# pudnax/voidin

Measured on AMD Instinct MI355X. Metric: M instances culled+compacted/sec, higher is better.
Workload: dtype f32; 1 GPU; configs[2]: 10M synthetic AABB instances, cull + prefix-sum compaction (BASELINE.md §3 distribution, model.rs camera); instances_per_gpu=10000000, instances_total=10000000, n_meshes=16, distribution=baseline, parallelism=single GPU

## Files before the change

### voidin_amd/csrc/cull.hip

```cpp
#include "vd_common.hpp"

#include <math.h>

namespace {

constexpr int kWave = 64;
constexpr int kBlock = 256;
constexpr int kWavesPerBlock = kBlock / kWave;
constexpr int kInstBytes = 144;
constexpr int kSlabBytes = kWave * kInstBytes;
constexpr int kChunksPerLane = kSlabBytes / (kWave * 16);



typedef unsigned int u32x4 __attribute__((ext_vector_type(4)));

struct CullCamera {
    float view[16];
    float frustum[4];
    float znear, zfar;
};

struct MeshRec { float mnx, mny, mnz; unsigned index_count; float mxx, mxy, mxz; unsigned base_index; int vertex_offset; };

// ... 276 lines not shown
    const float v0 = (0.5f - ny_hi * 0.5f) * H - 0.5f, v1 = (0.5f - ny_lo * 0.5f) * H + 0.5f;
    if (!(u1 >= 0.0f && v1 >= 0.0f && u0 < W && v0 < H)) return false;
    const unsigned x0 = (unsigned)floorf(fmaxf(u0, 0.0f)), x1 = (unsigned)floorf(fminf(u1, W - 1.0f));
    const unsigned y0 = (unsigned)floorf(fmaxf(v0, 0.0f)), y1 = (unsigned)floorf(fminf(v1, H - 1.0f));
    const unsigned span = max(x1 - x0, y1 - y0);
    const unsigned lvl = min(span ? 32u - (unsigned)__clz((int)span) : 0u, hz.n_levels - 1u);
    const float* t = hz.base + hz.off[lvl];
    const unsigned lw = ((hz.width - 1u) >> lvl) + 1u;
    const unsigned ax = x0 >> lvl, bx = x1 >> lvl, ay = y0 >> lvl, by = y1 >> lvl;
    const float h0 = fminf(t[(size_t)ay * lw + ax], t[(size_t)ay * lw + bx]);
    const float h1 = fminf(t[(size_t)by * lw + ax], t[(size_t)by * lw + bx]);
    const float hmin = fminf(h0, h1);
    const float depth = (cam.p32 - cam.p22 * dn) / dn;
    return depth < hmin;
}

__global__ __launch_bounds__(kBlock, 3) void occlusion_mask_kernel(OccCamera cam, HizView hz, const VdMeshInfo* __restrict__ meshes,
                                                                   unsigned n_mesh, const VdInstance* __restrict__ inst, unsigned n_inst,
                                                                   const vd_u64* __restrict__ mask_in, vd_u64* __restrict__ mask_out,
                                                                   unsigned n_wave_tiles) {
    extern __shared__ __attribute__((aligned(16))) char smem[];
    const unsigned lane = threadIdx.x & 63u, wave = threadIdx.x >> 6;
    char* slab = smem + wave * kSlabBytes;
    const unsigned waves_total = gridDim.x * kWavesPerBlock;
    u32x4 regs[kChunksPerLane];
    for (unsigned wt = blockIdx.x * kWavesPerBlock + wave; wt < n_wave_tiles; wt += waves_total) {
        const vd_u64 in = mask_in[wt];
        if (in == 0ull) {
            if (lane == 0) mask_out[wt] = 0ull;
            continue;
        }
        const size_t first = (size_t)wt * kWave;
        const unsigned n_valid = min(64u, n_inst - (unsigned)first);
        slab_fill<false>(inst, first, n_valid, lane, regs);
        slab_store(slab, lane, regs);
        vd_wave_lds_sync();
        const LaneInst li = slab_read(slab, lane);
        vd_wave_lds_sync();
        bool keep = false;
        if (lane < n_valid && ((in >> lane) & 1ull)) {
            const MeshRec m = load_mesh(meshes, min(li.mesh, n_mesh - 1u));
            keep = !is_occluded(cam, hz, m, li.T0, li.T1, li.T2, li.T3);
        }
        const unsigned long long b = __ballot(keep);
        if (lane == 0) mask_out[wt] = b;
    }
}

constexpr int kMaskRounds = 16;
template <typename IdT>
__global__ __launch_bounds__(kBlock, 3) void cull_mask_tiled_kernel(CullCamera cam, const VdMeshInfo* __restrict__ meshes,
                                                                     unsigned n_mesh, const VdInstance* __restrict__ inst,
                                                                     unsigned n_inst, vd_u64* __restrict__ mask,
                                                                     IdT* __restrict__ ids_out, unsigned n_tiles) {
    extern __shared__ __attribute__((aligned(16))) char smem[];
    const unsigned lane = threadIdx.x & 63u, wave = threadIdx.x >> 6;
    constexpr int kIdBytes = kMaskRounds * kWave * (int)sizeof(IdT);
    char* slab = smem + wave * (kSlabBytes + kIdBytes);
    IdT* s_ids = reinterpret_cast<IdT*>(slab + kSlabBytes);
    const unsigned waves_total = gridDim.x * kWavesPerBlock;
    auto valid_at = [&](size_t f) -> unsigned { return f < n_inst ? (unsigned)min((size_t)64, (size_t)n_inst - f) : 0u; };
    u32x4 regs[kChunksPerLane];
    for (unsigned t = blockIdx.x * kWavesPerBlock + wave; t < n_tiles; t += waves_total) {
        const size_t tile_first = (size_t)t * (kWave * kMaskRounds);
        slab_fill<true>(inst, tile_first, valid_at(tile_first), lane, regs);
        constexpr int kIdRows = kIdBytes / (kWave * 16);
        u32x4 old_ids[kIdRows];
        const size_t id_base0 = tile_first * sizeof(IdT);
        const bool full_tile = tile_first + (size_t)kWave * kMaskRounds <= (size_t)n_inst;
        if (full_tile) {
#pragma unroll
            for (int r = 0; r < kIdRows; ++r)
                old_ids[r] = *reinterpret_cast<const u32x4*>(reinterpret_cast<const char*>(ids_out) + id_base0 + (size_t)r * kWave * 16 + lane * 16u);
        }
        vd_u64 my_word = 0;
#pragma unroll 1
        for (int r = 0; r < kMaskRounds; ++r) {
            const size_t first = tile_first + (size_t)r * kWave;
            const unsigned n_valid = valid_at(first);
            slab_store(slab, lane, regs);
            if (r + 1 < kMaskRounds) slab_fill<true>(inst, first + kWave, valid_at(first + kWave), lane, regs);
            vd_wave_lds_sync();
            const LaneInst li = slab_read(slab, lane);
            vd_wave_lds_sync();
            const unsigned mid = min(li.mesh, n_mesh - 1u);
            const MeshRec m = load_mesh(meshes, mid);
            const bool vis = lane < n_valid && is_visible(cam, m, li.T0, li.T1, li.T2, li.T3);
            const unsigned long long b = __ballot(vis);
            if (lane == (unsigned)r) my_word = b;
            s_ids[r * kWave + lane] = (IdT)mid;
        }
        vd_wave_lds_sync();
        const size_t w0 = (size_t)t * kMaskRounds;
        const size_t n_words = ((size_t)n_inst + 63) / 64;
        if (lane < (unsigned)kMaskRounds && w0 + lane < n_words) mask[w0 + lane] = my_word;
        const size_t id_base = tile_first * sizeof(IdT);
        const size_t id_end = min((size_t)n_inst, tile_first + (size_t)kWave * kMaskRounds) * sizeof(IdT);
        char* gids = reinterpret_cast<char*>(ids_out);
        if (full_tile) {
#pragma unroll
            for (int r = 0; r < kIdRows; ++r) {
                const unsigned b0 = (unsigned)r * kWave * 16u + lane * 16u;
                const u32x4 nv = *reinterpret_cast<const u32x4*>(reinterpret_cast<const char*>(s_ids) + b0);
                const bool diff = nv.x != old_ids[r].x || nv.y != old_ids[r].y || nv.z != old_ids[r].z || nv.w != old_ids[r].w;
                if (__any(diff)) *reinterpret_cast<u32x4*>(gids + id_base + b0) = nv;
            }
        } else {
            for (unsigned b0 = lane * 16u; b0 < (unsigned)kIdBytes; b0 += kWave * 16u) {
                if (id_base + b0 + 16u <= id_end) {
                    *reinterpret_cast<u32x4*>(gids + id_base + b0) = *reinterpret_cast<const u32x4*>(reinterpret_cast<const char*>(s_ids) + b0);
                } else {
                    for (unsigned q = 0; q < 16u && id_base + b0 + q < id_end; ++q) gids[id_base + b0 + q] = reinterpret_cast<const char*>(s_ids)[b0 + q];
                }
            }
        }
        vd_wave_lds_sync();
    }
}

constexpr int kExpandGroup = 4;
constexpr int kExpandWords = 32;
constexpr int kChunkWords = kWavesPerBlock * kExpandWords;

constexpr int kScanBlock = 1024;
struct ScanState { unsigned done, epoch, pad[2]; };
__global__ __launch_bounds__(kScanBlock) void mask_scan_kernel(const vd_u64* __restrict__ mask, unsigned n_words, unsigned n_chunks,
                                                           vd_u64* chunk_entry, ScanState* state,
                                                           unsigned* __restrict__ out_count) {
    constexpr int kScanWaves = kScanBlock / kWave;
    __shared__ unsigned s_last, s_wave_sum[kScanWaves];
    const unsigned lane = threadIdx.x & 63u, wave = threadIdx.x >> 6;
    const unsigned ep = __hip_atomic_load(&state->epoch, VD_RLX_AGENT);
    const vd_u64 tag = (vd_u64)ep << 32;
    for (unsigned c = blockIdx.x * kScanWaves + wave; c < n_chunks; c += gridDim.x * kScanWaves) {
        const unsigned w = c * kChunkWords + lane;
        unsigned v = (w < n_words ? (unsigned)__popcll(mask[w]) : 0u) + (w + 64u < n_words ? (unsigned)__popcll(mask[w + 64u]) : 0u);
#pragma unroll
        for (int off = 32; off > 0; off >>= 1) v += __shfl_xor(v, off);
        if (lane == 0) __hip_atomic_store(&chunk_entry[c], tag | v, VD_RLX_AGENT);
    }
    __builtin_amdgcn_s_waitcnt(0);
    __syncthreads();
    if (threadIdx.x == 0) s_last = __hip_atomic_fetch_add(&state->done, 1u, VD_RLX_AGENT) == gridDim.x - 1u;
    __syncthreads();
    if (!s_last) return;
    const unsigned per = (n_chunks + kScanBlock - 1) / kScanBlock;
    const unsigned begin = min(threadIdx.x * per, n_chunks), end = min(begin + per, n_chunks);
    bool stuck = false;
    auto entry = [&](unsigned c) -> unsigned {
        vd_u64 e = __hip_atomic_load(&chunk_entry[c], VD_RLX_AGENT);
        unsigned spins = 0;
        while ((e >> 32) != (vd_u64)ep) {
            if (++spins > (1u << 22)) { stuck = true; return 0u; }
            __builtin_amdgcn_s_sleep(1);
            e = __hip_atomic_load(&chunk_entry[c], VD_RLX_AGENT);
        }
        return (unsigned)e;
    };
    unsigned sum = 0;
    for (unsigned c = begin; c < end; ++c) sum += entry(c);
    const bool any_stuck = __syncthreads_or(stuck ? 1 : 0) != 0;
    unsigned incl = sum;
#pragma unroll
    for (int off = 1; off < kWave; off <<= 1) {
        const unsigned t = __shfl_up(incl, off);
        if (lane >= (unsigned)off) incl += t;
    }
    if (lane == kWave - 1u) s_wave_sum[wave] = incl;
    __syncthreads();
    unsigned run = incl - sum;
    for (unsigned w = 0; w < wave; ++w) run += s_wave_sum[w];
    for (unsigned c = begin; c < end; ++c) {
        if (any_stuck) { chunk_entry[c] = tag | 0xffffffffu; continue; }
        const unsigned v = entry(c);
        chunk_entry[c] = tag | run;
        run += v;
    }
    if (threadIdx.x == kScanBlock - 1u) {
        *out_count = any_stuck ? 0xffffffffu : run;
        __hip_atomic_store(&state->done, 0u, VD_RLX_AGENT);
        __hip_atomic_store(&state->epoch, ep + 1u, VD_RLX_AGENT);
    }
}

template <typename IdT, bool TAB>
__global__ __launch_bounds__(kBlock) void expand_mask_kernel(const vd_u64* __restrict__ mask, unsigned n_words, unsigned wps,
                                                             unsigned shard_size, unsigned n_total, unsigned first_instance,
                                                             const IdT* __restrict__ mesh_ids,
                                                             const VdMeshInfo* __restrict__ meshes, unsigned n_mesh,
                                                             VdDrawIndexedIndirect* __restrict__ out,
                                                             const vd_u64* __restrict__ chunk_entry) {
    constexpr int kGroups = kExpandWords / kExpandGroup;
    constexpr unsigned kTab = TAB ? 512 : 1;
    __shared__ unsigned s_tab[kTab][3];
    constexpr int kStageBytes = kExpandGroup * 1280 + 32;
    __shared__ __attribute__((aligned(16))) char s_stage[kWavesPerBlock][kStageBytes];
    const unsigned lane = threadIdx.x & 63u, wave = threadIdx.x >> 6;
    const unsigned chunk = blockIdx.x;
    const unsigned cw0 = chunk * kChunkWords;
    const unsigned w0 = __builtin_amdgcn_readfirstlane(cw0 + wave * kExpandWords);
    unsigned base = (unsigned)chunk_entry[chunk];
    if (base == 0xffffffffu) return;
    unsigned before = 0;
    if (lane < wave * kExpandWords && cw0 + lane < n_words) before = (unsigned)__popcll(mask[cw0 + lane]);
    if (lane + 64u < wave * kExpandWords && cw0 + 64u + lane < n_words) before += (unsigned)__popcll(mask[cw0 + 64u + lane]);
    vd_u64 my_word = 0;
    if (lane < (unsigned)kExpandWords && w0 + lane < n_words) my_word = mask[w0 + lane];
    auto group_first = [&](unsigned wg, unsigned (&f)[kExpandGroup]) {
        unsigned shard = wg / wps, r = wg - shard * wps;
#pragma unroll
        for (int q = 0; q < kExpandGroup; ++q) {
            f[q] = shard * shard_size + 64u * r;
            if (++r >= wps) { r = 0u; ++shard; }
        }
    };
    unsigned ids[kExpandWords];
#pragma unroll
    for (int g = 0; g < kGroups; ++g) {
        const unsigned wg = w0 + g * kExpandGroup;
        unsigned f[kExpandGroup];
        group_first(wg, f);
#pragma unroll
        for (int q = 0; q < kExpandGroup; ++q) {
            const unsigned idx = f[q] + lane;
            ids[g * kExpandGroup + q] = (wg + q < n_words && idx < n_total) ? (unsigned)mesh_ids[idx] : 0u;
        }
    }
    if (TAB)
        for (unsigned i = threadIdx.x; i < n_mesh; i += kBlock) {
            s_tab[i][0] = meshes[i].index_count; s_tab[i][1] = meshes[i].base_index; s_tab[i][2] = (unsigned)meshes[i].vertex_offset;
        }
#pragma unroll
    for (int off = 32; off > 0; off >>= 1) before += __shfl_xor(before, off);
    base += before;
    __syncthreads();
    char* stage = s_stage[wave];
#pragma unroll
    for (int g = 0; g < kGroups; ++g) {
        const unsigned wg = w0 + g * kExpandGroup;
        vd_u64 m[kExpandGroup];
        unsigned cnt = 0;
#pragma unroll
        for (int q = 0; q < kExpandGroup; ++q) {
            const int k = g * kExpandGroup + q;
            const unsigned lo = __shfl((unsigned)my_word, k), hi = __shfl((unsigned)(my_word >> 32), k);
            m[q] = ((vd_u64)hi << 32) | lo;
            cnt += (unsigned)__popcll(m[q]);
        }
        if (cnt == 0u) continue;
        char* gbase = reinterpret_cast<char*>(out + base);
        const unsigned shift = (unsigned)(reinterpret_cast<uintptr_t>(gbase) & 15u);
        unsigned run = 0;
        unsigned first[kExpandGroup];
        group_first(wg, first);
#pragma unroll
        for (int q = 0; q < kExpandGroup; ++q) {
            unsigned mid = ids[g * kExpandGroup + q];
            if ((m[q] >> lane) & 1ull) {
                mid = min(mid, n_mesh - 1u);
                unsigned* o = reinterpret_cast<unsigned*>(stage + shift + 20u * (run + vd_mbcnt(m[q])));
                if (TAB) { o[0] = s_tab[mid][0]; o[2] = s_tab[mid][1]; o[3] = s_tab[mid][2]; }
                else { o[0] = meshes[mid].index_count; o[2] = meshes[mid].base_index; o[3] = (unsigned)meshes[mid].vertex_offset; }
                o[1] = 1u;
                o[4] = first_instance + first[q] + lane;
            }
            run += (unsigned)__popcll(m[q]);
        }
        vd_wave_lds_sync();
        const unsigned total = shift + 20u * cnt;
        char* g16 = gbase - shift;
        for (unsigned b0 = lane * 16u; b0 < total; b0 += kWave * 16u) {
            if (b0 >= shift && b0 + 16u <= total) {
                *reinterpret_cast<u32x4*>(g16 + b0) = *reinterpret_cast<const u32x4*>(stage + b0);
            } else {
                const unsigned lo_b = b0 > shift ? b0 : shift, hi_b = b0 + 16u < total ? b0 + 16u : total;
                for (unsigned b = lo_b; b < hi_b; b += 4u)
                    *reinterpret_cast<unsigned*>(g16 + b) = *reinterpret_cast<const unsigned*>(stage + b);
            }
        }
        vd_wave_lds_sync();
        base += cnt;
    }
}

template <bool DIRECT>
__global__ __launch_bounds__(kBlock) void expand_mask_u8_kernel(const vd_u64* __restrict__ mask, unsigned n_words, unsigned wps,
                                                                unsigned shard_size, unsigned n_total, unsigned first_instance,
                                                                const unsigned char* __restrict__ mesh_ids,
                                                                const VdMeshInfo* __restrict__ meshes, unsigned n_mesh,
                                                                VdDrawIndexedIndirect* __restrict__ out,
                                                                const vd_u64* __restrict__ chunk_entry) {
    constexpr int kGroups = kExpandWords / kExpandGroup;
    __shared__ __attribute__((aligned(16))) unsigned s_tab[256][4];
    constexpr int kStageBytes = DIRECT ? 16 : kExpandGroup * 1280 + 32;
    __shared__ __attribute__((aligned(16))) char s_stage[kWavesPerBlock][kStageBytes];
    const unsigned lane = threadIdx.x & 63u;
    const unsigned wave = __builtin_amdgcn_readfirstlane(threadIdx.x >> 6);
    const unsigned chunk = blockIdx.x;
    const unsigned cw0 = chunk * kChunkWords;
    const unsigned w0 = cw0 + wave * kExpandWords;
    unsigned base = (unsigned)chunk_entry[chunk];
    if (base == 0xffffffffu) return;
    unsigned before = 0;
    if (lane < wave * kExpandWords && cw0 + lane < n_words) before = (unsigned)__popcll(mask[cw0 + lane]);
    if (lane + 64u < wave * kExpandWords && cw0 + 64u + lane < n_words) before += (unsigned)__popcll(mask[cw0 + 64u + lane]);
    vd_u64 my_word = 0;
    if (lane < (unsigned)kExpandWords && w0 + lane < n_words) my_word = mask[w0 + lane];
    unsigned ids[kGroups];
    {
        const unsigned wl = w0 + (lane >> 4);
        unsigned shard = wl / wps, r = wl - shard * wps;
#pragma unroll
        for (int g = 0; g < kGroups; ++g) {
            const unsigned i0 = shard * shard_size + 64u * r + 4u * (lane & 15u);
            ids[g] = (wl + g * kExpandGroup < n_words && i0 < n_total) ? *reinterpret_cast<const unsigned*>(mesh_ids + i0) : 0u;
            r += kExpandGroup;
            if (r >= wps) { r -= wps; ++shard; }
        }
    }
    unsigned s_shard = w0 / wps, s_r = w0 - s_shard * wps;
    unsigned word_first = s_shard * shard_size + 64u * s_r;
    constexpr unsigned PF = DIRECT ? 0u : 32u;
    unsigned pf = 0;
    if (PF > 0) {
        const unsigned pw = (chunk + 8u * PF) * kChunkWords + (threadIdx.x >> 1);
        if (pw < n_words) {
            const unsigned ps = pw / wps;
            const unsigned pi = ps * shard_size + 64u * (pw - ps * wps) + 32u * (threadIdx.x & 1u);
            if (pi + 32u <= n_total) {
                const u32x4 a = *reinterpret_cast<const u32x4*>(mesh_ids + pi), b = *reinterpret_cast<const u32x4*>(mesh_ids + pi + 16u);
                pf = a.x ^ a.w ^ b.x ^ b.w;
            }
            if ((threadIdx.x & 1u) == 0u) pf ^= (unsigned)mask[pw];
        }
    }
    if (threadIdx.x < n_mesh) {
        const VdMeshInfo mi = meshes[threadIdx.x];
        s_tab[threadIdx.x][0] = mi.index_count; s_tab[threadIdx.x][1] = 1u;
        s_tab[threadIdx.x][2] = mi.base_index;  s_tab[threadIdx.x][3] = (unsigned)mi.vertex_offset;
    }
#pragma unroll
    for (int off = 32; off > 0; off >>= 1) before += __shfl_xor(before, off);
    base = __builtin_amdgcn_readfirstlane(base + before);
    __syncthreads();
    const unsigned max_mid = n_mesh - 1u;
    const unsigned inst_lane = first_instance + lane;
    const unsigned id_shift = 8u * (lane & 3u);
    char* stage = s_stage[wave];
#pragma unroll
    for (int g = 0; g < kGroups; ++g) {
        vd_u64 m[kExpandGroup];
        unsigned cnt = 0;
#pragma unroll
        for (int q = 0; q < kExpandGroup; ++q) {
            const int k = g * kExpandGroup + q;
            const unsigned lo = __builtin_amdgcn_readlane((unsigned)my_word, k), hi = __builtin_amdgcn_readlane((unsigned)(my_word >> 32), k);
            m[q] = ((vd_u64)hi << 32) | lo;
            cnt += (unsigned)__popcll(m[q]);
        }
        unsigned wf[kExpandGroup];
#pragma unroll
        for (int q = 0; q < kExpandGroup; ++q) {
            wf[q] = word_first;
            if (++s_r >= wps) { s_r = 0u; ++s_shard; }
            word_first = s_shard * shard_size + 64u * s_r;
        }
        if (cnt == 0u) continue;
        if (DIRECT) {
            unsigned run = base;
#pragma unroll
            for (int q = 0; q < kExpandGroup; ++q) {
                const unsigned v = (unsigned)__shfl((int)ids[g], q * 16 + (int)(lane >> 2));
                const unsigned mid = min((v >> id_shift) & 0xffu, max_mid);
                if (__builtin_amdgcn_inverse_ballot_w64(m[q])) {
                    unsigned* o = reinterpret_cast<unsigned*>(out + (run + vd_mbcnt(m[q])));
                    typedef u32x4 __attribute__((aligned(4))) u32x4_a4;
                    *reinterpret_cast<u32x4_a4*>(o) = *reinterpret_cast<const u32x4*>(s_tab[mid]);
                    o[4] = inst_lane + wf[q];
                }
                run += (unsigned)__popcll(m[q]);
            }
        } else {
            char* gbase = reinterpret_cast<char*>(out + base);
            const unsigned shift = (unsigned)(reinterpret_cast<uintptr_t>(gbase) & 15u);
            unsigned run = 0;
#pragma unroll
            for (int q = 0; q < kExpandGroup; ++q) {
                const unsigned v = (unsigned)__shfl((int)ids[g], q * 16 + (int)(lane >> 2));
                const unsigned mid = min((v >> id_shift) & 0xffu, max_mid);
                if (__builtin_amdgcn_inverse_ballot_w64(m[q])) {
                    unsigned* o = reinterpret_cast<unsigned*>(stage + shift + 20u * (run + vd_mbcnt(m[q])));
                    const u32x4 c = *reinterpret_cast<const u32x4*>(s_tab[mid]);
                    o[0] = c.x; o[1] = c.y; o[2] = c.z; o[3] = c.w;
                    o[4] = inst_lane + wf[q];
                }
                run += (unsigned)__popcll(m[q]);
            }
// ... 129 lines not shown
        if (__builtin_amdgcn_inverse_ballot_w64(m)) out[base + vd_mbcnt(m)] = inst_lane + 64u * (unsigned)k;
        base += (unsigned)__popcll(m);
    }
}

template <typename IdT>
__global__ __launch_bounds__(kBlock) void indices_to_draws_kernel(const unsigned* __restrict__ indices, unsigned n_indices,
                                                                  const IdT* __restrict__ mesh_ids, unsigned n_total,
                                                                  const VdMeshInfo* __restrict__ meshes, unsigned n_mesh,
                                                                  VdDrawIndexedIndirect* __restrict__ out) {
    constexpr unsigned kTab = 512;
    __shared__ __attribute__((aligned(16))) unsigned s_tab[kTab][4];
    const bool tab = n_mesh <= kTab;
    if (tab)
        for (unsigned i = threadIdx.x; i < n_mesh; i += kBlock) {
            s_tab[i][0] = meshes[i].index_count; s_tab[i][1] = 1u;
            s_tab[i][2] = meshes[i].base_index;  s_tab[i][3] = (unsigned)meshes[i].vertex_offset;
        }
    __syncthreads();
    for (unsigned k = blockIdx.x * kBlock + threadIdx.x; k < n_indices; k += gridDim.x * kBlock) {
        const unsigned i = indices[k];
        const unsigned mid = min((unsigned)mesh_ids[min(i, n_total - 1u)], n_mesh - 1u);
        u32x4 c;
        if (tab) c = *reinterpret_cast<const u32x4*>(s_tab[mid]);
        else { c.x = meshes[mid].index_count; c.y = 1u; c.z = meshes[mid].base_index; c.w = (unsigned)meshes[mid].vertex_offset; }
        unsigned* o = reinterpret_cast<unsigned*>(out + k);
        typedef u32x4 __attribute__((aligned(4))) u32x4_a4;
        *reinterpret_cast<u32x4_a4*>(o) = c;
        o[4] = i;
    }
}

static int launch_mask_scan(VdCtx* ctx, const vd_u64* d_mask, unsigned n_words, unsigned* d_out_count, vd_u64** out_entries) {
    const unsigned n_chunks = (n_words + kChunkWords - 1) / kChunkWords;
    const size_t need = sizeof(ScanState) + (size_t)n_chunks * 8;
    if (need > ctx->expand_state_bytes || !ctx->expand_state) {
        int rc = vd_ensure(ctx, &ctx->expand_state, &ctx->expand_state_bytes, need);
        if (rc) return rc;
        VD_HIP_CHECK(ctx, hipMemsetAsync(ctx->expand_state, 0, ctx->expand_state_bytes, ctx->stream));
        VD_HIP_CHECK(ctx, hipMemsetD32Async(reinterpret_cast<hipDeviceptr_t>(reinterpret_cast<char*>(ctx->expand_state) + offsetof(ScanState, epoch)), 1, 1, ctx->stream));
    }
    ScanState* state = reinterpret_cast<ScanState*>(ctx->expand_state);
    vd_u64* entries = reinterpret_cast<vd_u64*>(reinterpret_cast<char*>(ctx->expand_state) + sizeof(ScanState));
    unsigned sblocks = (n_chunks + 15u) / 16u;
    if (sblocks > (unsigned)ctx->num_cus * 2u) sblocks = (unsigned)ctx->num_cus * 2u;
    hipLaunchKernelGGL(mask_scan_kernel, dim3(sblocks), dim3(kScanBlock), 0, ctx->stream, d_mask, n_words, n_chunks, entries, state,
                       d_out_count);
    *out_entries = entries;
    return VD_OK;
}

static int launch_expand(VdCtx* ctx, const vd_u64* d_mask, unsigned n_words, unsigned wps, unsigned shard_size,
                         unsigned n_total, unsigned first_instance, const void* d_ids, unsigned id_bytes,
                         const VdMeshInfo* d_meshes, unsigned n_mesh, VdDrawIndexedIndirect* d_out, unsigned* d_out_count) {
    const unsigned n_chunks = (n_words + kChunkWords - 1) / kChunkWords;
    vd_u64* offsets;
    int rc_scan = launch_mask_scan(ctx, d_mask, n_words, d_out_count, &offsets);
    if (rc_scan) return rc_scan;
    const bool one_shard = wps >= n_words;
    const bool tab = n_mesh <= 512u;
    const bool fast = id_bytes == 1u && n_mesh <= 256u && (one_shard || (shard_size % 4u == 0u && wps >= (unsigned)kExpandGroup)) &&
                      (reinterpret_cast<uintptr_t>(d_ids) & 3u) == 0u;
    if (fast) {
#define VD_EXPAND_U8(D)                                                                                                   \
        hipLaunchKernelGGL((expand_mask_u8_kernel<D>), dim3(n_chunks), dim3(kBlock), 0, ctx->stream, d_mask, n_words, wps,  \
                           shard_size, n_total, first_instance, reinterpret_cast<const unsigned char*>(d_ids), d_meshes,    \
                           n_mesh, d_out, offsets)
        if (n_total <= (12u << 20)) VD_EXPAND_U8(true);
        else VD_EXPAND_U8(false);
#undef VD_EXPAND_U8
        return VD_OK;
    }
#define VD_EXPAND(IdT, T)                                                                                               \
    hipLaunchKernelGGL((expand_mask_kernel<IdT, T>), dim3(n_chunks), dim3(kBlock), 0, ctx->stream, d_mask, n_words, wps,  \
                       shard_size, n_total, first_instance, reinterpret_cast<const IdT*>(d_ids), d_meshes, n_mesh, d_out,    \
                       offsets)
    if (id_bytes == 1u) { if (tab) VD_EXPAND(unsigned char, true); else VD_EXPAND(unsigned char, false); }
    else if (id_bytes == 2u) { if (tab) VD_EXPAND(unsigned short, true); else VD_EXPAND(unsigned short, false); }
    else { if (tab) VD_EXPAND(unsigned, true); else VD_EXPAND(unsigned, false); }
#undef VD_EXPAND
    return VD_OK;
}

__global__ __launch_bounds__(kBlock) void pad_tail_kernel(VdDrawIndexedIndirect* __restrict__ out,
                                                          const unsigned* __restrict__ count, unsigned n) {
    const unsigned c = *count;
    const size_t begin = (c > n ? (size_t)0 : (size_t)c) * 5u, end = (size_t)n * 5u;
    unsigned* o = reinterpret_cast<unsigned*>(out);
    if (begin >= end) return;
    const size_t gid = (size_t)blockIdx.x * kBlock + threadIdx.x, gsz = (size_t)gridDim.x * kBlock;
    const size_t mis = (reinterpret_cast<uintptr_t>(o + begin) >> 2) & 3u;
    const size_t head = min(end - begin, (4u - mis) & 3u);
    const size_t quads = (end - begin - head) >> 2;
    const size_t tail_first = begin + head + quads * 4u;
    if (gid < head) o[begin + gid] = 0u;
    if (gid < end - tail_first) o[tail_first + gid] = 0u;
    u32x4* q = reinterpret_cast<u32x4*>(o + begin + head);
    const u32x4 z = {0u, 0u, 0u, 0u};
    for (size_t i = gid; i < quads; i += gsz) __builtin_nontemporal_store(z, q + i);
}

constexpr int kCompactPerThread = 8;
constexpr int kCompactTile = kBlock * kCompactPerThread;

__global__ __launch_bounds__(kBlock) void compact_draws_kernel(const VdDrawIndexedIndirect* __restrict__ in, unsigned n,
                                                               VdDrawIndexedIndirect* __restrict__ out,
                                                               unsigned* __restrict__ out_count, vd_u64* tile_state,
                                                               vd_u64* ticket_counter, unsigned n_tiles, unsigned* fault_host) {
    __shared__ unsigned s_ticket, s_epoch, s_wave_total[kWavesPerBlock], s_tile_excl;
    const unsigned lane = threadIdx.x & 63u, wave = threadIdx.x >> 6;
    if (threadIdx.x == 0) s_ticket = vd_take_ticket(ticket_counter, n_tiles, &s_epoch);
    __syncthreads();
    const unsigned tile = s_ticket, epoch = s_epoch;
    if (tile >= n_tiles) return;
    if (tile == 0u && threadIdx.x == 0) { __hip_atomic_store(out_count, VD_SCAN_STUCK, VD_RLX_AGENT); __threadfence(); }
    const size_t wave_first = (size_t)tile * kCompactTile + (size_t)wave * (kWave * kCompactPerThread);
    unsigned long long masks[kCompactPerThread];
    unsigned wave_total = 0;
    const unsigned* in32 = reinterpret_cast<const unsigned*>(in);
#pragma unroll
    for (int r = 0; r < kCompactPerThread; ++r) {
        const size_t i = wave_first + (size_t)r * kWave + lane;
        const bool keep = i < n && in32[i * 5u + 1u] == 1u;
        masks[r] = __ballot(keep);
        wave_total += (unsigned)__popcll(masks[r]);
    }
    if (lane == 0) s_wave_total[wave] = wave_total;
    __syncthreads();
    if (wave == 0) {
        unsigned tile_total = 0;
#pragma unroll
        for (int w = 0; w < kWavesPerBlock; ++w) tile_total += s_wave_total[w];
        const unsigned excl = vd_lookback(tile_state, epoch, tile, tile_total);
// ... 31 lines not shown
    const bool live = idx < n_inst;
    float4* t4 = reinterpret_cast<float4*>(inst[live ? idx : 0u].transform);
    float4 v = make_float4(0.0f, 0.0f, 0.0f, 0.0f);
    if (live) v = t4[col];
    const float t14 = quad_bcast<3>(v.z);
    const bool pos = t14 > -15.0f;
    const float c = pos ? rz.c_pos : rz.c_neg, s = pos ? rz.s_pos : rz.s_neg;
    float4 o;
    o.x = ((c * v.x + -s * v.y) + 0.0f * v.z) + 0.0f * v.w;
    o.y = ((s * v.x + c * v.y) + 0.0f * v.z) + 0.0f * v.w;
    o.z = ((0.0f * v.x + 0.0f * v.y) + 1.0f * v.z) + 0.0f * v.w;
    o.w = ((0.0f * v.x + 0.0f * v.y) + 0.0f * v.z) + 1.0f * v.w;
    if (live) t4[col] = o;
    if (fix_inverse) {
        float4* i4 = reinterpret_cast<float4*>(inst[live ? idx : 0u].inv_transform);
        float4 w = make_float4(0.0f, 0.0f, 0.0f, 0.0f);
        if (live) w = i4[col];
        const float4 I0 = make_float4(quad_bcast<0>(w.x), quad_bcast<0>(w.y), quad_bcast<0>(w.z), quad_bcast<0>(w.w));
        const float4 I1 = make_float4(quad_bcast<1>(w.x), quad_bcast<1>(w.y), quad_bcast<1>(w.z), quad_bcast<1>(w.w));
        const float4 I2 = make_float4(quad_bcast<2>(w.x), quad_bcast<2>(w.y), quad_bcast<2>(w.z), quad_bcast<2>(w.w));
        const float4 I3 = make_float4(quad_bcast<3>(w.x), quad_bcast<3>(w.y), quad_bcast<3>(w.z), quad_bcast<3>(w.w));
        const float b0 = col == 0u ? c : (col == 1u ? s : 0.0f);
        const float b1 = col == 0u ? -s : (col == 1u ? c : 0.0f);
        const float b2 = col == 2u ? 1.0f : 0.0f, b3 = col == 3u ? 1.0f : 0.0f;
        float4 r;
        r.x = ((I0.x * b0 + I1.x * b1) + I2.x * b2) + I3.x * b3;
        r.y = ((I0.y * b0 + I1.y * b1) + I2.y * b2) + I3.y * b3;
        r.z = ((I0.z * b0 + I1.z * b1) + I2.z * b2) + I3.z * b3;
        r.w = ((I0.w * b0 + I1.w * b1) + I2.w * b2) + I3.w * b3;
        if (live) i4[col] = r;
    }
}

CullCamera make_cam(const VdCameraUniform* c) {
    CullCamera k;
    memcpy(k.view, c->view, sizeof(k.view));
    memcpy(k.frustum, c->frustum, sizeof(k.frustum));
    k.znear = c->znear;
    k.zfar = c->zfar;
    return k;
}

}

extern "C" {

int vd_cull_emit_dev(VdCtx* ctx, const VdCameraUniform* camera, const VdMeshInfo* d_meshes, uint32_t n_mesh,
                     const VdInstance* d_instances, uint32_t n_inst, VdDrawIndexedIndirect* d_out) {
    VdDeviceGuard vd_guard_(ctx);
    return vd_cull_emit_shard_dev(ctx, camera, d_meshes, n_mesh, d_instances, n_inst, 0u, d_out);
}

static int launch_mask_pass(VdCtx* ctx, const VdCameraUniform* camera, const VdMeshInfo* d_meshes, uint32_t n_mesh,
                            const VdInstance* d_instances, uint32_t n_inst, vd_u64** out_mask, void** out_ids, unsigned* out_id_bytes) {
    const unsigned n_words = (n_inst + 63u) / 64u;
    const unsigned id_bytes = n_mesh <= 256u ? 1u : (n_mesh <= 65536u ? 2u : 4u);
    const size_t need = (size_t)n_words * 8 + (size_t)n_inst * id_bytes + 512;
    int rc = vd_ensure(ctx, &ctx->scratch, &ctx->scratch_bytes, need);
    if (rc) return rc;
    vd_u64* d_mask = reinterpret_cast<vd_u64*>(ctx->scratch);
    void* d_ids = reinterpret_cast<char*>(ctx->scratch) + (((size_t)n_words * 8 + 255) & ~(size_t)255);
    vd_time_begin(ctx);
    const unsigned n_mt = (n_inst + kWave * kMaskRounds - 1) / (kWave * kMaskRounds);
    unsigned mb = (n_mt + kWavesPerBlock - 1) / kWavesPerBlock;
    if (mb > (unsigned)ctx->num_cus * 3u) mb = (unsigned)ctx->num_cus * 3u;
#define VD_SPLIT(IdT)                                                                                              \
    hipLaunchKernelGGL(cull_mask_tiled_kernel<IdT>, dim3(mb), dim3(kBlock),                                        \
                       kWavesPerBlock * (kSlabBytes + kMaskRounds * kWave * (int)sizeof(IdT)),                     \
                       ctx->stream, make_cam(camera), d_meshes, n_mesh, d_instances, n_inst, d_mask,               \
                       reinterpret_cast<IdT*>(d_ids), n_mt)
    if (id_bytes == 1u) VD_SPLIT(unsigned char);
    else if (id_bytes == 2u) VD_SPLIT(unsigned short);
    else VD_SPLIT(unsigned);
#undef VD_SPLIT
    vd_time_mid(ctx);
    *out_mask = d_mask; *out_ids = d_ids; *out_id_bytes = id_bytes;
    return VD_OK;
}

int vd_cull_emit_shard_dev(VdCtx* ctx, const VdCameraUniform* camera, const VdMeshInfo* d_meshes, uint32_t n_mesh,
                           const VdInstance* d_instances, uint32_t n_inst, uint32_t first_instance,
                           VdDrawIndexedIndirect* d_out) {
    VdDeviceGuard vd_guard_(ctx);
    if (!ctx) return VD_ERR_INVALID_ARG;
    if (!camera || !d_meshes || n_mesh == 0) VD_FAIL(ctx, VD_ERR_INVALID_ARG, "vd_cull_emit: null camera/meshes or n_mesh == 0");
    if (n_inst == 0) return VD_OK;
    if (!d_instances || !d_out) VD_FAIL(ctx, VD_ERR_INVALID_ARG, "vd_cull_emit: null instances/out");
    if (ctx->option(VD_OPT_CULL_VARIANT, 0) <= 0 && n_inst >= ctx->split_min) {
        vd_u64* d_mask; void* d_ids; unsigned id_bytes;
        int rc = launch_mask_pass(ctx, camera, d_meshes, n_mesh, d_instances, n_inst, &d_mask, &d_ids, &id_bytes);
        if (rc) return rc;
        const unsigned quads = (n_inst + 3u) / 4u;
        unsigned eb = (quads + kBlock - 1) / kBlock;
        if (eb > (unsigned)ctx->num_cus * 16u) eb = (unsigned)ctx->num_cus * 16u;
#define VD_EMIT(IdT) hipLaunchKernelGGL(emit_from_mask_kernel<IdT>, dim3(eb), dim3(kBlock), 0, ctx->stream, d_mask,               \
                                        reinterpret_cast<const IdT*>(d_ids), d_meshes, n_mesh, n_inst, first_instance, d_out)
        if (id_bytes == 1u) {
            const unsigned n_words = (n_inst + 63u) / 64u;
            hipLaunchKernelGGL(emit_all_u8_kernel, dim3((n_words + kChunkWords - 1) / kChunkWords), dim3(kBlock), 0, ctx->stream, d_mask,
                               n_words, n_inst, first_instance, reinterpret_cast<const unsigned char*>(d_ids), d_meshes, n_mesh, d_out);
        } else if (id_bytes == 2u) VD_EMIT(unsigned short); else VD_EMIT(unsigned);
#undef VD_EMIT
        vd_time_end(ctx);
        VD_HIP_CHECK(ctx, hipGetLastError());
        return VD_OK;
    }
    const unsigned n_wave_tiles = (n_inst + kWave - 1) / kWave;
    unsigned blocks = (n_wave_tiles + kWavesPerBlock - 1) / kWavesPerBlock;
    const unsigned cap = (unsigned)ctx->num_cus * 4u;
    if (blocks > cap) blocks = cap;
    vd_time_begin(ctx);
    hipLaunchKernelGGL(emit_draws_kernel, dim3(blocks), dim3(kBlock), kWavesPerBlock * kSlabBytes, ctx->stream,
                       make_cam(camera), d_meshes, n_mesh, d_instances, n_inst, d_out, n_wave_tiles, first_instance);
    vd_time_end(ctx);
    VD_HIP_CHECK(ctx, hipGetLastError());
    return VD_OK;
}

int vd_cull_compact_dev(VdCtx* ctx, const VdCameraUniform* camera, const VdMeshInfo* d_meshes, uint32_t n_mesh,
                        const VdInstance* d_instances, uint32_t n_inst, VdDrawIndexedIndirect* d_out,
                        uint32_t* d_out_count, int pad_tail) {
    VdDeviceGuard vd_guard_(ctx);
    return vd_cull_compact_shard_dev(ctx, camera, d_meshes, n_mesh, d_instances, n_inst, 0u, d_out, d_out_count, pad_tail);
}

int vd_cull_compact_shard_dev(VdCtx* ctx, const VdCameraUniform* camera, const VdMeshInfo* d_meshes, uint32_t n_mesh,
                              const VdInstance* d_instances, uint32_t n_inst, uint32_t first_instance,
                              VdDrawIndexedIndirect* d_out, uint32_t* d_out_count, int pad_tail) {
    VdDeviceGuard vd_guard_(ctx);
    if (!ctx) return VD_ERR_INVALID_ARG;
    if (!camera || !d_meshes || n_mesh == 0 || !d_out_count)
        VD_FAIL(ctx, VD_ERR_INVALID_ARG, "vd_cull_compact: null camera/meshes/count or n_mesh == 0");
    if (n_inst == 0) {
        VD_HIP_CHECK(ctx, hipMemsetAsync(d_out_count, 0, 4, ctx->stream));
        return VD_OK;
    }
    if (!d_instances || !d_out) VD_FAIL(ctx, VD_ERR_INVALID_ARG, "vd_cull_compact: null instances/out");
    const int variant = (int)ctx->option(VD_OPT_CULL_VARIANT, 0);
    vd_u64* ticket; vd_u64* states;
    int rc = vd_scan_check_fault(ctx);
    if (rc) return rc;
    if (variant <= 0 && n_inst >= ctx->split_min) {
        vd_u64* d_mask; void* d_ids; unsigned id_bytes;
        rc = launch_mask_pass(ctx, camera, d_meshes, n_mesh, d_instances, n_inst, &d_mask, &d_ids, &id_bytes);
        if (rc) return rc;
        const unsigned n_words = (n_inst + 63u) / 64u;
        rc = launch_expand(ctx, d_mask, n_words, n_words, n_inst, n_inst, first_instance, d_ids, id_bytes, d_meshes, n_mesh,
                           d_out, d_out_count);
        if (rc) return rc;
        vd_time_end(ctx);
        if (pad_tail) {
            unsigned pblocks = (unsigned)ctx->num_cus * 4u;
            hipLaunchKernelGGL(pad_tail_kernel, dim3(pblocks), dim3(kBlock), 0, ctx->stream, d_out, d_out_count, n_inst);
        }
        VD_HIP_CHECK(ctx, hipGetLastError());
        return VD_OK;
    }
#define VD_LAUNCH_COMPACT(R)                                                                                     \
    do {                                                                                                         \
        const unsigned n_tiles = (n_inst + kBlock * (R) - 1) / (kBlock * (R));                                   \
        rc = vd_scan_scratch(ctx, n_tiles, &ticket, &states, true);                                              \
        if (rc) return rc;                                                                                       \
        hipLaunchKernelGGL((cull_compact_kernel<R>), dim3(n_tiles), dim3(kBlock), (compact_lds_bytes<R>()),      \
                           ctx->stream, make_cam(camera), d_meshes, n_mesh, d_instances, n_inst, d_out,          \
                           d_out_count, states, ticket, n_tiles, first_instance, vd_scan_fault_word(ctx));       \
    } while (0)
    const int rounds = variant > 0 ? variant : (n_inst >= (4u << 20) ? 32 : (n_inst >= (5u << 18) ? 16 : (n_inst >= 600000u ? 8 : (n_inst >= 192000u ? 4 : (n_inst >= 48000u ? 2 : 1)))));
    switch (rounds) {
        case 1: VD_LAUNCH_COMPACT(1); break;
        case 2: VD_LAUNCH_COMPACT(2); break;
        case 4: VD_LAUNCH_COMPACT(4); break;
        case 8: VD_LAUNCH_COMPACT(8); break;
        case 16: VD_LAUNCH_COMPACT(16); break;
        default: VD_LAUNCH_COMPACT(32); break;
    }
#undef VD_LAUNCH_COMPACT
    vd_time_end(ctx);
    if (pad_tail) {
        unsigned blocks = (unsigned)ctx->num_cus * 4u;
        hipLaunchKernelGGL(pad_tail_kernel, dim3(blocks), dim3(kBlock), 0, ctx->stream, d_out, d_out_count, n_inst);
    }
    VD_HIP_CHECK(ctx, hipGetLastError());
    return VD_OK;
}

int vd_cull_mask_dev(VdCtx* ctx, const VdCameraUniform* camera, const VdMeshInfo* d_meshes, uint32_t n_mesh,
                     const VdInstance* d_instances, uint32_t n_inst, uint64_t* d_mask) {
    VdDeviceGuard vd_guard_(ctx);
    if (!ctx) return VD_ERR_INVALID_ARG;
    if (!camera || !d_meshes || n_mesh == 0) VD_FAIL(ctx, VD_ERR_INVALID_ARG, "vd_cull_mask: null camera/meshes or n_mesh == 0");
    if (n_inst == 0) return VD_OK;
    if (!d_instances || !d_mask) VD_FAIL(ctx, VD_ERR_INVALID_ARG, "vd_cull_mask: null instances/mask");
    const unsigned n_wave_tiles = (n_inst + kWave - 1) / kWave;
    unsigned blocks = (n_wave_tiles + kWavesPerBlock - 1) / kWavesPerBlock;
    const unsigned cap = (unsigned)ctx->num_cus * 4u;
    if (blocks > cap) blocks = cap;
    vd_time_begin(ctx);
    hipLaunchKernelGGL(cull_mask_kernel<unsigned>, dim3(blocks), dim3(kBlock), kWavesPerBlock * kSlabBytes, ctx->stream, make_cam(camera),
                       d_meshes, n_mesh, d_instances, n_inst, reinterpret_cast<vd_u64*>(d_mask), (unsigned*)nullptr, n_wave_tiles);
    vd_time_end(ctx);
    VD_HIP_CHECK(ctx, hipGetLastError());
// ... 224 lines not shown
```

Baseline: 38770 M instances/s.

## Replace separate mask scan with per-tile survivor counts reduced in expand kernel

The cull mask kernel now also writes a per-tile survivor count (popcount of the tile's ballot words, reduced across lanes). In the single-shard compaction path, the expand kernels no longer depend on the separate mask-scan launch with its decoupled-lookback chunk offsets. Instead, each block recomputes its base offset by summing all tile counts before its chunk, and the last block writes the total count. This removes one kernel launch and the serial scan dependency, but every expand block redundantly reads a prefix of the tile-count array, so that work grows roughly quadratically with instance count.

```diff
diff --git a/voidin_amd/csrc/cull.hip b/voidin_amd/csrc/cull.hip
--- a/voidin_amd/csrc/cull.hip
+++ b/voidin_amd/csrc/cull.hip
@@ -352,7 +352,8 @@
 __global__ __launch_bounds__(kBlock, 3) void cull_mask_tiled_kernel(CullCamera cam, const VdMeshInfo* __restrict__ meshes,
                                                                      unsigned n_mesh, const VdInstance* __restrict__ inst,
                                                                      unsigned n_inst, vd_u64* __restrict__ mask,
-                                                                     IdT* __restrict__ ids_out, unsigned n_tiles) {
+                                                                     IdT* __restrict__ ids_out, unsigned* __restrict__ tile_count,
+                                                                     unsigned n_tiles) {
     extern __shared__ __attribute__((aligned(16))) char smem[];
     const unsigned lane = threadIdx.x & 63u, wave = threadIdx.x >> 6;
     constexpr int kIdBytes = kMaskRounds * kWave * (int)sizeof(IdT);
@@ -394,6 +395,10 @@
         const size_t w0 = (size_t)t * kMaskRounds;
         const size_t n_words = ((size_t)n_inst + 63) / 64;
         if (lane < (unsigned)kMaskRounds && w0 + lane < n_words) mask[w0 + lane] = my_word;
+        unsigned survivors = (unsigned)__popcll(my_word);
+#pragma unroll
+        for (int off = kMaskRounds / 2; off > 0; off >>= 1) survivors += __shfl_xor(survivors, off);
+        if (lane == 0u) tile_count[t] = survivors;
         const size_t id_base = tile_first * sizeof(IdT);
         const size_t id_end = min((size_t)n_inst, tile_first + (size_t)kWave * kMaskRounds) * sizeof(IdT);
         char* gids = reinterpret_cast<char*>(ids_out);
@@ -483,14 +488,40 @@
     }
 }
 
-template <typename IdT, bool TAB>
+constexpr int kChunkTiles = kChunkWords / kMaskRounds;
+
+__device__ __forceinline__ unsigned tile_prefix_partial(const unsigned* __restrict__ tile_count, unsigned n_before) {
+    constexpr unsigned kBatch = 4;
+    unsigned sum = 0;
+    for (unsigned i0 = threadIdx.x * 4u; i0 < n_before; i0 += kBatch * kBlock * 4u) {
+        u32x4 v[kBatch];
+#pragma unroll
+        for (unsigned k = 0; k < kBatch; ++k) {
+            const unsigned i = i0 + k * kBlock * 4u;
+            v[k] = *reinterpret_cast<const u32x4*>(tile_count + (i < n_before ? i : i0));
+        }
+#pragma unroll
+        for (unsigned k = 0; k < kBatch; ++k) {
+            const unsigned i = i0 + k * kBlock * 4u;
+            sum += (i < n_before ? v[k].x : 0u) + (i + 1u < n_before ? v[k].y : 0u) + (i + 2u < n_before ? v[k].z : 0u) +
+                   (i + 3u < n_before ? v[k].w : 0u);
+        }
+    }
+#pragma unroll
+    for (int off = 32; off > 0; off >>= 1) sum += __shfl_xor(sum, off);
+    return sum;
+}
+
+template <typename IdT, bool TAB, bool TILES>
 __global__ __launch_bounds__(kBlock) void expand_mask_kernel(const vd_u64* __restrict__ mask, unsigned n_words, unsigned wps,
                                                              unsigned shard_size, unsigned n_total, unsigned first_instance,
                                                              const IdT* __restrict__ mesh_ids,
                                                              const VdMeshInfo* __restrict__ meshes, unsigned n_mesh,
                                                              VdDrawIndexedIndirect* __restrict__ out,
-                                                             const vd_u64* __restrict__ chunk_entry) {
+                                                             const vd_u64* __restrict__ chunk_entry,
+                                                             const unsigned* __restrict__ tile_count, unsigned* __restrict__ out_count) {
     constexpr int kGroups = kExpandWords / kExpandGroup;
+    __shared__ unsigned s_prefix[kWavesPerBlock];
     constexpr unsigned kTab = TAB ? 512 : 1;
     __shared__ unsigned s_tab[kTab][3];
     constexpr int kStageBytes = kExpandGroup * 1280 + 32;
@@ -499,8 +530,14 @@
     const unsigned chunk = blockIdx.x;
     const unsigned cw0 = chunk * kChunkWords;
     const unsigned w0 = __builtin_amdgcn_readfirstlane(cw0 + wave * kExpandWords);
-    unsigned base = (unsigned)chunk_entry[chunk];
-    if (base == 0xffffffffu) return;
+    unsigned base = 0;
+    if (TILES) {
+        const unsigned part = tile_prefix_partial(tile_count, chunk * kChunkTiles);
+        if (lane == 0) s_prefix[wave] = part;
+    } else {
+        base = (unsigned)chunk_entry[chunk];
+        if (base == 0xffffffffu) return;
+    }
     unsigned before = 0;
     if (lane < wave * kExpandWords && cw0 + lane < n_words) before = (unsigned)__popcll(mask[cw0 + lane]);
     if (lane + 64u < wave * kExpandWords && cw0 + 64u + lane < n_words) before += (unsigned)__popcll(mask[cw0 + 64u + lane]);
@@ -534,6 +571,16 @@
     for (int off = 32; off > 0; off >>= 1) before += __shfl_xor(before, off);
     base += before;
     __syncthreads();
+    if (TILES) {
+#pragma unroll
+        for (int w = 0; w < kWavesPerBlock; ++w) base += s_prefix[w];
+        if (chunk == gridDim.x - 1u && wave == kWavesPerBlock - 1u) {
+            unsigned mine = (unsigned)__popcll(my_word);
+#pragma unroll
+            for (int off = 32; off > 0; off >>= 1) mine += __shfl_xor(mine, off);
+            if (lane == 0) *out_count = base + mine;
+        }
+    }
     char* stage = s_stage[wave];
 #pragma unroll
     for (int g = 0; g < kGroups; ++g) {
@@ -583,14 +630,16 @@
     }
 }
 
-template <bool DIRECT>
+template <bool DIRECT, bool TILES>
 __global__ __launch_bounds__(kBlock) void expand_mask_u8_kernel(const vd_u64* __restrict__ mask, unsigned n_words, unsigned wps,
                                                                 unsigned shard_size, unsigned n_total, unsigned first_instance,
                                                                 const unsigned char* __restrict__ mesh_ids,
                                                                 const VdMeshInfo* __restrict__ meshes, unsigned n_mesh,
                                                                 VdDrawIndexedIndirect* __restrict__ out,
-                                                                const vd_u64* __restrict__ chunk_entry) {
+                                                                const vd_u64* __restrict__ chunk_entry,
+                                                                const unsigned* __restrict__ tile_count, unsigned* __restrict__ out_count) {
     constexpr int kGroups = kExpandWords / kExpandGroup;
+    __shared__ unsigned s_prefix[kWavesPerBlock];
     __shared__ __attribute__((aligned(16))) unsigned s_tab[256][4];
     constexpr int kStageBytes = DIRECT ? 16 : kExpandGroup * 1280 + 32;
     __shared__ __attribute__((aligned(16))) char s_stage[kWavesPerBlock][kStageBytes];
@@ -599,8 +648,14 @@
     const unsigned chunk = blockIdx.x;
     const unsigned cw0 = chunk * kChunkWords;
     const unsigned w0 = cw0 + wave * kExpandWords;
-    unsigned base = (unsigned)chunk_entry[chunk];
-    if (base == 0xffffffffu) return;
+    unsigned base = 0;
+    if (TILES) {
+        const unsigned part = tile_prefix_partial(tile_count, chunk * kChunkTiles);
+        if (lane == 0) s_prefix[wave] = part;
+    } else {
+        base = (unsigned)chunk_entry[chunk];
+        if (base == 0xffffffffu) return;
+    }
     unsigned before = 0;
     if (lane < wave * kExpandWords && cw0 + lane < n_words) before = (unsigned)__popcll(mask[cw0 + lane]);
     if (lane + 64u < wave * kExpandWords && cw0 + 64u + lane < n_words) before += (unsigned)__popcll(mask[cw0 + 64u + lane]);
@@ -643,6 +698,17 @@
     for (int off = 32; off > 0; off >>= 1) before += __shfl_xor(before, off);
     base = __builtin_amdgcn_readfirstlane(base + before);
     __syncthreads();
+    if (TILES) {
+#pragma unroll
+        for (int w = 0; w < kWavesPerBlock; ++w) base += s_prefix[w];
+        base = __builtin_amdgcn_readfirstlane(base);
+        if (chunk == gridDim.x - 1u && wave == kWavesPerBlock - 1u) {
+            unsigned mine = (unsigned)__popcll(my_word);
+#pragma unroll
+            for (int off = 32; off > 0; off >>= 1) mine += __shfl_xor(mine, off);
+            if (lane == 0) *out_count = base + mine;
+        }
+    }
     const unsigned max_mid = n_mesh - 1u;
     const unsigned inst_lane = first_instance + lane;
     const unsigned id_shift = 8u * (lane & 3u);
@@ -878,33 +944,39 @@
 
 static int launch_expand(VdCtx* ctx, const vd_u64* d_mask, unsigned n_words, unsigned wps, unsigned shard_size,
                          unsigned n_total, unsigned first_instance, const void* d_ids, unsigned id_bytes,
-                         const VdMeshInfo* d_meshes, unsigned n_mesh, VdDrawIndexedIndirect* d_out, unsigned* d_out_count) {
+                         const VdMeshInfo* d_meshes, unsigned n_mesh, VdDrawIndexedIndirect* d_out, unsigned* d_out_count,
+                         const unsigned* d_tile_count = nullptr) {
     const unsigned n_chunks = (n_words + kChunkWords - 1) / kChunkWords;
-    vd_u64* offsets;
-    int rc_scan = launch_mask_scan(ctx, d_mask, n_words, d_out_count, &offsets);
-    if (rc_scan) return rc_scan;
+    vd_u64* offsets = nullptr;
+    if (!d_tile_count) {
+        int rc_scan = launch_mask_scan(ctx, d_mask, n_words, d_out_count, &offsets);
+        if (rc_scan) return rc_scan;
+    }
     const bool one_shard = wps >= n_words;
     const bool tab = n_mesh <= 512u;
     const bool fast = id_bytes == 1u && n_mesh <= 256u && (one_shard || (shard_size % 4u == 0u && wps >= (unsigned)kExpandGroup)) &&
                       (reinterpret_cast<uintptr_t>(d_ids) & 3u) == 0u;
     if (fast) {
-#define VD_EXPAND_U8(D)                                                                                                   \
-        hipLaunchKernelGGL((expand_mask_u8_kernel<D>), dim3(n_chunks), dim3(kBlock), 0, ctx->stream, d_mask, n_words, wps,  \
-                           shard_size, n_total, first_instance, reinterpret_cast<const unsigned char*>(d_ids), d_meshes,    \
-                           n_mesh, d_out, offsets)
-        if (n_total <= (12u << 20)) VD_EXPAND_U8(true);
-        else VD_EXPAND_U8(false);
+#define VD_EXPAND_U8(D, T)                                                                                                  \
+        hipLaunchKernelGGL((expand_mask_u8_kernel<D, T>), dim3(n_chunks), dim3(kBlock), 0, ctx->stream, d_mask, n_words, wps, \
+                           shard_size, n_total, first_instance, reinterpret_cast<const unsigned char*>(d_ids), d_meshes,      \
+                           n_mesh, d_out, offsets, d_tile_count, d_out_count)
+        const bool direct = n_total <= (12u << 20);
+        if (d_tile_count) { if (direct) VD_EXPAND_U8(true, true); else VD_EXPAND_U8(false, true); }
+        else { if (direct) VD_EXPAND_U8(true, false); else VD_EXPAND_U8(false, false); }
 #undef VD_EXPAND_U8
         return VD_OK;
     }
-#define VD_EXPAND(IdT, T)                                                                                               \
-    hipLaunchKernelGGL((expand_mask_kernel<IdT, T>), dim3(n_chunks), dim3(kBlock), 0, ctx->stream, d_mask, n_words, wps,  \
+#define VD_EXPAND_T(IdT, T, S)                                                                                             \
+    hipLaunchKernelGGL((expand_mask_kernel<IdT, T, S>), dim3(n_chunks), dim3(kBlock), 0, ctx->stream, d_mask, n_words, wps, \
                        shard_size, n_total, first_instance, reinterpret_cast<const IdT*>(d_ids), d_meshes, n_mesh, d_out,    \
-                       offsets)
+                       offsets, d_tile_count, d_out_count)
+#define VD_EXPAND(IdT, T) do { if (d_tile_count) VD_EXPAND_T(IdT, T, true); else VD_EXPAND_T(IdT, T, false); } while (0)
     if (id_bytes == 1u) { if (tab) VD_EXPAND(unsigned char, true); else VD_EXPAND(unsigned char, false); }
     else if (id_bytes == 2u) { if (tab) VD_EXPAND(unsigned short, true); else VD_EXPAND(unsigned short, false); }
     else { if (tab) VD_EXPAND(unsigned, true); else VD_EXPAND(unsigned, false); }
 #undef VD_EXPAND
+#undef VD_EXPAND_T
     return VD_OK;
 }
 
@@ -1042,29 +1114,33 @@
 }
 
 static int launch_mask_pass(VdCtx* ctx, const VdCameraUniform* camera, const VdMeshInfo* d_meshes, uint32_t n_mesh,
-                            const VdInstance* d_instances, uint32_t n_inst, vd_u64** out_mask, void** out_ids, unsigned* out_id_bytes) {
+                            const VdInstance* d_instances, uint32_t n_inst, vd_u64** out_mask, void** out_ids, unsigned* out_id_bytes,
+                            unsigned** out_tile_count) {
     const unsigned n_words = (n_inst + 63u) / 64u;
     const unsigned id_bytes = n_mesh <= 256u ? 1u : (n_mesh <= 65536u ? 2u : 4u);
-    const size_t need = (size_t)n_words * 8 + (size_t)n_inst * id_bytes + 512;
+    const unsigned n_mt = (n_inst + kWave * kMaskRounds - 1) / (kWave * kMaskRounds);
+    const size_t ids_off = ((size_t)n_words * 8 + 255) & ~(size_t)255;
+    const size_t counts_off = (ids_off + (size_t)n_inst * id_bytes + 15) & ~(size_t)15;
+    const size_t need = counts_off + (((size_t)n_mt + 3) & ~(size_t)3) * 4 + 512;
     int rc = vd_ensure(ctx, &ctx->scratch, &ctx->scratch_bytes, need);
     if (rc) return rc;
     vd_u64* d_mask = reinterpret_cast<vd_u64*>(ctx->scratch);
-    void* d_ids = reinterpret_cast<char*>(ctx->scratch) + (((size_t)n_words * 8 + 255) & ~(size_t)255);
+    void* d_ids = reinterpret_cast<char*>(ctx->scratch) + ids_off;
+    unsigned* d_counts = reinterpret_cast<unsigned*>(reinterpret_cast<char*>(ctx->scratch) + counts_off);
     vd_time_begin(ctx);
-    const unsigned n_mt = (n_inst + kWave * kMaskRounds - 1) / (kWave * kMaskRounds);
     unsigned mb = (n_mt + kWavesPerBlock - 1) / kWavesPerBlock;
     if (mb > (unsigned)ctx->num_cus * 3u) mb = (unsigned)ctx->num_cus * 3u;
 #define VD_SPLIT(IdT)                                                                                              \
     hipLaunchKernelGGL(cull_mask_tiled_kernel<IdT>, dim3(mb), dim3(kBlock),                                        \
                        kWavesPerBlock * (kSlabBytes + kMaskRounds * kWave * (int)sizeof(IdT)),                     \
                        ctx->stream, make_cam(camera), d_meshes, n_mesh, d_instances, n_inst, d_mask,               \
-                       reinterpret_cast<IdT*>(d_ids), n_mt)
+                       reinterpret_cast<IdT*>(d_ids), d_counts, n_mt)
     if (id_bytes == 1u) VD_SPLIT(unsigned char);
     else if (id_bytes == 2u) VD_SPLIT(unsigned short);
     else VD_SPLIT(unsigned);
 #undef VD_SPLIT
     vd_time_mid(ctx);
-    *out_mask = d_mask; *out_ids = d_ids; *out_id_bytes = id_bytes;
+    *out_mask = d_mask; *out_ids = d_ids; *out_id_bytes = id_bytes; *out_tile_count = d_counts;
     return VD_OK;
 }
 
@@ -1077,8 +1153,8 @@
     if (n_inst == 0) return VD_OK;
     if (!d_instances || !d_out) VD_FAIL(ctx, VD_ERR_INVALID_ARG, "vd_cull_emit: null instances/out");
     if (ctx->option(VD_OPT_CULL_VARIANT, 0) <= 0 && n_inst >= ctx->split_min) {
-        vd_u64* d_mask; void* d_ids; unsigned id_bytes;
-        int rc = launch_mask_pass(ctx, camera, d_meshes, n_mesh, d_instances, n_inst, &d_mask, &d_ids, &id_bytes);
+        vd_u64* d_mask; void* d_ids; unsigned id_bytes; unsigned* d_tile_count;
+        int rc = launch_mask_pass(ctx, camera, d_meshes, n_mesh, d_instances, n_inst, &d_mask, &d_ids, &id_bytes, &d_tile_count);
         if (rc) return rc;
         const unsigned quads = (n_inst + 3u) / 4u;
         unsigned eb = (quads + kBlock - 1) / kBlock;
@@ -1131,12 +1207,12 @@
     int rc = vd_scan_check_fault(ctx);
     if (rc) return rc;
     if (variant <= 0 && n_inst >= ctx->split_min) {
-        vd_u64* d_mask; void* d_ids; unsigned id_bytes;
-        rc = launch_mask_pass(ctx, camera, d_meshes, n_mesh, d_instances, n_inst, &d_mask, &d_ids, &id_bytes);
+        vd_u64* d_mask; void* d_ids; unsigned id_bytes; unsigned* d_tile_count;
+        rc = launch_mask_pass(ctx, camera, d_meshes, n_mesh, d_instances, n_inst, &d_mask, &d_ids, &id_bytes, &d_tile_count);
         if (rc) return rc;
         const unsigned n_words = (n_inst + 63u) / 64u;
         rc = launch_expand(ctx, d_mask, n_words, n_words, n_inst, n_inst, first_instance, d_ids, id_bytes, d_meshes, n_mesh,
-                           d_out, d_out_count);
+                           d_out, d_out_count, d_tile_count);
         if (rc) return rc;
         vd_time_end(ctx);
         if (pad_tail) {
```

Result: faster. 39580 M instances/s (median of 6 runs) (+2.1%).
